# OChicken/GPQHE

Measured on AMD Instinct MI355X. Metric: ciphertext he_mul/sec (RNS core: tensor 30 limbs + key-switch 45 limbs), N=2^16, higher is better.
Workload: dtype u64; 1 GPU; he_mul RNS core, n=2^16, dimA=30, dimB=45, batch=64 ciphertexts per GPU (BASELINE configs[2]); he_rescale has no RNS-domain work in the reference; batch_per_gpu=64, total_batch=64, chunk=32, parallelism=ciphertext-per-GPU x1, no data-path collective, launcher=single process

## Files before the change

### gpqhe_amd/csrc/engine.hip

```cpp
#include "../../include/gpqhe_hip.h"
#include "engine_internal.hpp"
#include "ntt_kernels.hpp"

#include <cmath>
#include <cstdlib>
#include <cstdarg>
#include <cstdio>
#include <cstring>
#include <new>
#include <type_traits>

using namespace gpq;

static thread_local char g_err[512] = "";

int gpq_fail(int code, const char *fmt, ...) {
  va_list ap;
  va_start(ap, fmt);
  vsnprintf(g_err, sizeof g_err, fmt, ap);
  va_end(ap);
  return code;
}
extern "C" const char *gpq_last_error(void) { return g_err; }

// ... 399 lines not shown
    for (int i = 0; i < GPQ_MAX_SLABS; ++i) { if (a.src[i]) a.src[i] += shift; if (a.dst[i]) a.dst[i] += shift; }
    if (evk0) *evk0 += shift;
    if (evk1) *evk1 += shift;
    if (a.zflag) a.zflag += limbs;
  };
  int rc;
  if constexpr (WIDE)
    if (e_wide > lo) { if ((rc = f(TwW{}, a, e_wide - lo))) return rc; advance(e_wide - lo); }
  if (e_split > e_wide) { if ((rc = f(TwS{}, a, e_split - e_wide))) return rc; advance(e_split - e_wide); }
  if (hi > e_split && (rc = f(uint64_t{}, a, hi - e_split))) return rc;
  return GPQ_OK;
}

template <typename F>
static inline void with_nt(unsigned nt, F f) {
  if (nt) f(std::true_type{});
  else f(std::false_type{});
}

template <typename TW_, int LOW_, bool NT_>
struct Mid8Inst { using TW = TW_; static constexpr int LOW = LOW_; static constexpr bool NT = NT_; };
template <typename F>
static int launch_mid8(const gpq_ctx *c, const PassArgs &m, unsigned limbs, const uint64_t **evk0, const uint64_t **evk1, int slot, hipStream_t s, F launch) {
  return for_limb_ranges<true>(c, m, limbs, evk0, evk1, [&](auto tag, const PassArgs &a, unsigned nl) {
    using TW = decltype(tag);
    ProfScope prof(c, slot, s);
    with_nt(a.nt, [&](auto nt) {
      constexpr bool NT = decltype(nt)::value;
      if (c->low9) launch(Mid8Inst<TW, 9, NT>{}, a, nl);
      else launch(Mid8Inst<TW, 8, NT>{}, a, nl);
    });
    return (int)GPQ_OK;
  });
}
template <typename K>
static int launch_mid8(const gpq_ctx *c, const PassArgs &m, unsigned limbs, unsigned polys, int slot, hipStream_t s, K kernel) {
  return launch_mid8(c, m, limbs, nullptr, nullptr, slot, s, [&](auto inst, const PassArgs &a, unsigned nl) {
    hipLaunchKernelGGL(kernel(inst), dim3(c->n >> 11, polys, nl), dim3(CONTIG_WAVES * 64), 0, s, a);
  });
}
template <typename K, typename... Tail>
static int launch_keyswitch_mid8(const gpq_ctx *c, KeyswitchArgs m, unsigned limbs, unsigned polys, int slot, hipStream_t s, K kernel, Tail... tail) {
  return launch_mid8(c, m.p, limbs, &m.evk0, &m.evk1, slot, s, [&](auto inst, const PassArgs &a, unsigned nl) {
    KeyswitchArgs ka{a, m.evk0, m.evk1};
    const dim3 block(CONTIG_WAVES * 64);
    if (polys / 2) hipLaunchKernelGGL(kernel(inst, std::true_type{}), dim3(c->n >> 11, polys / 2, nl), block, 0, s, ka, 0u, tail...);
    if (polys & 1) hipLaunchKernelGGL(kernel(inst, std::false_type{}), dim3(c->n >> 11, 1, nl), block, 0, s, ka, polys - 1, tail...);
  });
}

template <int M1, int EL, bool INV, bool CANON, typename TW, int CW = 8>
int launch_strided_t(const PassArgs &a, unsigned gy, unsigned gz, hipStream_t s) {
  using G = StridedGeom<M1, EL>;
  with_nt(a.nt, [&](auto nt) {
    hipLaunchKernelGGL((strided_pass<M1, EL, INV, CANON, TW, CW, decltype(nt)::value>), dim3((1u << CW) >> G::CB, gy, gz), dim3(G::T), 0, s, a);
  });
  return GPQ_OK;
}

template <bool INV>
int launch_strided(const gpq_ctx *c, const PassArgs &args, unsigned dim, unsigned polys, hipStream_t s) {
  return for_limb_ranges<true>(c, args, dim, nullptr, nullptr, [&](auto tag, const PassArgs &a, unsigned limbs) {
    using TW = decltype(tag);
    ProfScope prof(c, INV ? GPQ_K_STRIDED_INV : GPQ_K_STRIDED_FWD, s);
    switch (c->logn) {
      case 13: return launch_strided_t<5, 4, INV, false, TW>(a, polys * a.nslab, limbs, s);
      case 14: return launch_strided_t<6, 4, INV, false, TW>(a, polys * a.nslab, limbs, s);
      case 15: return launch_strided_t<7, 4, INV, false, TW>(a, polys * a.nslab, limbs, s);
      case 16: return launch_strided_t<8, 4, INV, false, TW>(a, polys * a.nslab, limbs, s);
      case 17:
        return launch_strided_t<8, 4, INV, false, TW, 9>(a, polys * a.nslab, limbs, s);
    }
    return gpq_fail(GPQ_ERR_INVALID, "two-pass NTT needs 13 <= logn <= 17 (got %u)", c->logn);
  });
}

template <bool INV>
int launch_contig(const gpq_ctx *c, const PassArgs &args, unsigned dim, unsigned polys, hipStream_t s) {
  if (args.nslab != 1) return gpq_fail(GPQ_ERR_INVALID, "contig_pass walks one slab");
  return for_limb_ranges<true>(c, args, dim, nullptr, nullptr, [&](auto tag, const PassArgs &a, unsigned limbs) {
    using TW = decltype(tag);
    ProfScope prof(c, INV ? GPQ_K_CONTIG_INV : GPQ_K_CONTIG_FWD, s);
    if (c->low9) {
      const dim3 grid9(c->n >> 11, (polys + CONTIG8_POLYS - 1) / CONTIG8_POLYS, limbs);
      with_nt(a.nt, [&](auto nt) { hipLaunchKernelGGL((contig_pass8<INV, TW, 9, decltype(nt)::value>), grid9, dim3(CONTIG_WAVES * 64), 0, s, a, polys); });
      return (int)GPQ_OK;
    }
    const dim3 grid(c->n >> 12, (polys + CONTIG_POLYS - 1) / CONTIG_POLYS, limbs);
    with_nt(a.nt, [&](auto nt) { hipLaunchKernelGGL((contig_pass<INV, TW, decltype(nt)::value>), grid, dim3(CONTIG_WAVES * 64), 0, s, a, polys); });
    return (int)GPQ_OK;
  });
}

template <bool INV>
int launch_small(const gpq_ctx *c, const PassArgs &args, unsigned dim, unsigned polys, hipStream_t s) {
  return for_limb_ranges<false>(c, args, dim, nullptr, nullptr, [&](auto tag, const PassArgs &a, unsigned limbs) {
    using TW = decltype(tag);
    const dim3 grid(1, polys * a.nslab, limbs);
    ProfScope prof(c, GPQ_K_SMALL, s);
    hipLaunchKernelGGL((small_ntt<INV, TW>), grid, dim3(256), 0, s, a);
    return (int)GPQ_OK;
  });
}

inline bool two_pass(const gpq_ctx *c) { return c->logn > (unsigned)SMALL_MAX_LOGN; }

int after_launch(const char *who) {
  hipError_t e = hipGetLastError();
// ... 574 lines not shown
```

### gpqhe_amd/csrc/ntt_kernels.hpp

```cpp
#pragma once
#include "modarith.hpp"
#include "tables.hpp"

namespace gpq {

template <bool NT> __device__ __forceinline__ uint64_t slab_ld(const uint64_t *p) {
  if constexpr (NT) return __builtin_nontemporal_load(p);
  else return *p;
}
template <bool NT> __device__ __forceinline__ void slab_st(uint64_t *p, uint64_t v) {
  if constexpr (NT) __builtin_nontemporal_store(v, p);
  else *p = v;
}


constexpr int tw_count(int EL, int BHI, int BLO) { return (1 << (EL - BLO)) - (1 << (EL - BHI - 1)); }

constexpr int tw_off(int EL, int BHI, int b) { return (1 << (EL - b - 1)) - (1 << (EL - BHI - 1)); }

template <int EL, int BHI, int B, int BLO, bool UNIFORM, int NTW, typename TW>
__device__ __forceinline__ void load_tw_bits(TW (&tw)[NTW], unsigned ibase, int rs, unsigned logn,
                                             const TW *__restrict__ w) {
  const int sh = rs + B + 1;
  const TW *wp = w + (1u << (logn - sh)) + (UNIFORM ? 0u : (ibase >> sh));
#pragma unroll
  for (int j = 0; j < (1 << (EL - B - 1)); ++j) tw[tw_off(EL, BHI, B) + j] = wp[j];
  if constexpr (B > BLO) load_tw_bits<EL, BHI, B - 1, BLO, UNIFORM>(tw, ibase, rs, logn, w);
}

template <int EL, int BHI, int BLO, bool UNIFORM, typename TW>
__device__ __forceinline__ void load_tw(TW (&tw)[tw_count(EL, BHI, BLO)], unsigned ibase, int rs, unsigned logn,
                                        const TW *__restrict__ w) {
  load_tw_bits<EL, BHI, BHI, BLO, UNIFORM>(tw, ibase, rs, logn, w);
}

template <int S, typename TW>
__device__ __forceinline__ void ct_stage(uint64_t &x, uint64_t &y, const TW &w, const PrimeK &k) { ct_bfly(x, y, w, k); }
template <int S>
__device__ __forceinline__ void ct_stage(uint64_t &x, uint64_t &y, const TwW &w, const PrimeK &k) { ct_bfly_wide<(S & 1) == 0>(x, y, w, k); }

template <int EL, int BHI, int B, int BLO, int RS, int NTW, typename TW>
__device__ __forceinline__ void ct_bits(uint64_t (&x)[1 << EL], const TW (&tw)[NTW], const PrimeK &k) {
#pragma unroll
  for (int e = 0; e < (1 << EL); ++e)
    if (!(e & (1 << B))) ct_stage<RS + B>(x[e], x[e + (1 << B)], tw[tw_off(EL, BHI, B) + (e >> (B + 1))], k);
  if constexpr (B > BLO) ct_bits<EL, BHI, B - 1, BLO, RS>(x, tw, k);
}
template <int EL, int BHI, int BLO, int RS, typename TW>
__device__ __forceinline__ void ct_group(uint64_t (&x)[1 << EL], const TW (&tw)[tw_count(EL, BHI, BLO)],
                                         const PrimeK &k) {
  ct_bits<EL, BHI, BHI, BLO, RS>(x, tw, k);
}

template <bool BOTH_PRODUCT_LEGS, typename TW>
__device__ __forceinline__ void gs_stage(uint64_t &x, uint64_t &y, const TW &w, const PrimeK &k) { gs_bfly(x, y, w, k); }
template <bool BOTH_PRODUCT_LEGS>
__device__ __forceinline__ void gs_stage(uint64_t &x, uint64_t &y, const TwW &w, const PrimeK &k) { gs_bfly_wide<!BOTH_PRODUCT_LEGS>(x, y, w, k); }

template <int EL, int BHI, int B, int NTH, bool CANON_IN, int NTW, typename TW>
__device__ __forceinline__ void gs_bits(uint64_t (&x)[1 << EL], const TW (&tw)[NTW], const PrimeK &k) {
#pragma unroll
  for (int e = 0; e < (1 << EL); ++e)
    if (!(e & (1 << B))) {
      const TW &w = tw[tw_off(EL, BHI, B) + (e >> (B + 1))];
      if ((CANON_IN && NTH < 2) || (NTH > 0 && B > 0 && ((e >> (B > 0 ? B - 1 : 0)) & 1))) gs_stage<true>(x[e], x[e + (1 << B)], w, k);
      else gs_stage<false>(x[e], x[e + (1 << B)], w, k);
    }
// ... 40 lines not shown
template <> struct TwTraits<TwS> {
  __device__ static __forceinline__ const TwS *table(const PassArgs &a, bool inv) { return inv ? a.winvs : a.ws; }
  __device__ static __forceinline__ uint64_t canon_fwd(uint64_t x, const PrimeK &k) { return canon_fold(x, k.p, k.c); }
  __device__ static __forceinline__ uint64_t canon_inv(uint64_t x, const PrimeK &k) { return canon4(x, k); }
  __device__ static __forceinline__ uint64_t inv_from4(uint64_t x, const PrimeK &k) { return csub2(x, k); }
  __device__ static __forceinline__ uint64_t inv_from8(uint64_t x, const PrimeK &k) { return csub2(csub4(x, k), k); }
  __device__ static __forceinline__ uint64_t left(uint64_t x, const PrimeK &k) { return csub2(csub4(x, k), k); }
  __device__ static __forceinline__ uint64_t right(uint64_t x, const PrimeK &) { return x; }
};

template <> struct LastK<TwW> : LastK<TwS> {
  __device__ __forceinline__ explicit LastK(const LimbTab &t) : LastK<TwS>(t) {}
};
__device__ __forceinline__ void gs_last(uint64_t &x, uint64_t &y, const LastK<TwW> &t, const PrimeK &k) {
  const uint64_t s = x + y;
  const uint64_t d = x + k.p4 - y;
  x = csub1(mulmod_split(s, t.ninv, k), k);
  y = csub1(mulmod_split(d, t.winv1_ninv, k), k);
}
template <> struct TwTraits<TwW> {
  __device__ static __forceinline__ const TwW *table(const PassArgs &a, bool inv) { return reinterpret_cast<const TwW *>(inv ? a.winvs : a.ws); }
  __device__ static __forceinline__ uint64_t canon_fwd(uint64_t x, const PrimeK &k) { return canon_fold(x, k.p, k.c); }
  __device__ static __forceinline__ uint64_t canon_inv(uint64_t x, const PrimeK &k) { return canon4(x, k); }
  __device__ static __forceinline__ uint64_t inv_from4(uint64_t x, const PrimeK &) { return x; }
  __device__ static __forceinline__ uint64_t inv_from8(uint64_t x, const PrimeK &k) { return csub4(x, k); }
  __device__ static __forceinline__ uint64_t left(uint64_t x, const PrimeK &k) { return csub4(x, k); }
  __device__ static __forceinline__ uint64_t right(uint64_t x, const PrimeK &) { return x; }
};

__device__ __forceinline__ void zero_watch(uint32_t &m, uint64_t x) {
  const uint32_t t = (uint32_t)x | (uint32_t)(x >> 32);
  m = t < m ? t : m;
}
__device__ __forceinline__ void zero_note(const PassArgs &a, uint32_t m, unsigned poly, unsigned limb_in_launch) {
  if (m == 0 && a.zflag) atomicOr(a.zflag + (size_t)poly * a.zstride + limb_in_launch, 1u);
}

#ifndef GPQ_STRIDED_CB
#define GPQ_STRIDED_CB 4
#endif
template <int M1, int EL>
struct StridedGeom {
  static constexpr int CB = M1 <= 8 ? GPQ_STRIDED_CB : 4;
  static constexpr int C = 1 << CB;
  static constexpr int E = 1 << EL;
  static constexpr int T = 1 << (M1 + CB - EL);
  static constexpr int S2 = M1 - EL;
  static constexpr int BB = S2 > 0 ? S2 - 1 : 0;
  static constexpr int LDS_ELEMS = (1 << (M1 + CB)) + ((S2 > 0) ? (C << S2) : 0);
  __device__ static __forceinline__ unsigned pad(unsigned l) { return l + ((l >> (EL + CB)) << CB); }
};

template <int M1, int EL, bool INV, bool CANON_OUT, typename TW, int CW = 8, bool NT = false>
__global__ __launch_bounds__((StridedGeom<M1, EL>::T)) void strided_pass(PassArgs a) {
  using G = StridedGeom<M1, EL>;
  constexpr int E = G::E;
  constexpr unsigned logn = M1 + CW;
  __shared__ uint64_t lds[G::S2 > 0 ? G::LDS_ELEMS : 1];

  unsigned bx = blockIdx.x, by = blockIdx.y, bz = blockIdx.z;
  if (!INV) {
    const unsigned lin = blockIdx.x + gridDim.x * (blockIdx.y + gridDim.y * blockIdx.z), tot = gridDim.x * gridDim.y * gridDim.z;
    const unsigned logical = (lin & 7) * (tot >> 3) + (lin >> 3);
    bx = logical % gridDim.x; by = (logical / gridDim.x) % gridDim.y; bz = logical / (gridDim.x * gridDim.y);
  }
  const unsigned limb = a.limb0 + bz;
  const LimbTab &tab = a.tabs[limb];
  const PrimeK k = pin_consts(tab.k);
  const LastK<TW> last(tab);
  const TW *__restrict__ wt = TwTraits<TW>::table(a, INV) + ((size_t)limb << logn);
  const unsigned slab = by % a.nslab, poly = by / a.nslab;
  const size_t off = (size_t)poly * a.poly_stride + ((size_t)bz << logn);
  const uint64_t *__restrict__ src = a.src[slab] + off;
  uint64_t *__restrict__ dst = a.dst[slab] + off;

  const unsigned tid = threadIdx.x;
  constexpr int CB = G::CB;
  const unsigned col = (bx << CB) + (tid & (G::C - 1));
  const unsigned q = tid >> CB;
  const unsigned iA = (q << CW) + col, iB = (q << (EL + CW)) + col;
  constexpr unsigned strideA = 1u << (G::S2 + CW), strideB = 1u << CW;
  uint64_t x[E];
  TW twB[tw_count(EL, G::BB, 0)];

  if (!INV) {
    TW twA[tw_count(EL, EL - 1, 0)];
#pragma unroll
    for (int e = 0; e < E; ++e) x[e] = slab_ld<NT>(&src[iA + e * strideA]);
    load_tw<EL, EL - 1, 0, true>(twA, iA, G::S2 + CW, logn, wt);
    if (G::S2 > 0) load_tw<EL, G::BB, 0, false>(twB, iB, CW, logn, wt);
    ct_group<EL, EL - 1, 0, G::S2 + CW>(x, twA, k);
    if (G::S2 > 0) {
#pragma unroll
      for (int e = 0; e < E; ++e) lds[G::pad(tid + e * G::T)] = x[e];
      __syncthreads();
#pragma unroll
      for (int e = 0; e < E; ++e) x[e] = lds[G::pad((q << (EL + CB)) + (e << CB) + (tid & (G::C - 1)))];
      ct_group<EL, G::BB, 0, CW>(x, twB, k);
#pragma unroll
      for (int e = 0; e < E; ++e) slab_st<NT>(&dst[iB + e * strideB], CANON_OUT ? TwTraits<TW>::canon_fwd(x[e], k) : x[e]);
    } else {
#pragma unroll
      for (int e = 0; e < E; ++e) slab_st<NT>(&dst[iA + e * strideA], CANON_OUT ? TwTraits<TW>::canon_fwd(x[e], k) : x[e]);
    }
  } else {
    TW twA[tw_count(EL, (EL > 1 ? EL - 2 : 0), 0)];
    if (G::S2 > 0) {
#pragma unroll
      for (int e = 0; e < E; ++e) x[e] = slab_ld<NT>(&src[iB + e * strideB]);
      load_tw<EL, G::BB, 0, false>(twB, iB, CW, logn, wt);
      if (EL > 1) load_tw<EL, (EL > 1 ? EL - 2 : 0), 0, true>(twA, iA, G::S2 + CW, logn, wt);
      gs_group<EL, G::BB, 0>(x, twB, k);
#pragma unroll
      for (int e = 0; e < E; ++e) lds[G::pad((q << (EL + CB)) + (e << CB) + (tid & (G::C - 1)))] = x[e];
      __syncthreads();
#pragma unroll
      for (int e = 0; e < E; ++e) x[e] = lds[G::pad(tid + e * G::T)];
    } else {
#pragma unroll
      for (int e = 0; e < E; ++e) x[e] = slab_ld<NT>(&src[iA + e * strideA]);
      if (EL > 1) load_tw<EL, (EL > 1 ? EL - 2 : 0), 0, true>(twA, iA, G::S2 + CW, logn, wt);
    }
    if (EL > 1) gs_group<EL, (EL > 1 ? EL - 2 : 0), 0>(x, twA, k);
#pragma unroll
    for (int e = 0; e < E / 2; ++e) gs_last(x[e], x[e + E / 2], last, k);
#pragma unroll
    for (int e = 0; e < E; ++e) slab_st<NT>(&dst[iA + e * strideA], x[e]);
  }
}

constexpr int CONTIG_WAVES = 4;
constexpr int CONTIG_LDS_PER_WAVE = 1024 + 64;

__device__ __forceinline__ void wave_lds_sync() {
  __builtin_amdgcn_fence(__ATOMIC_RELEASE, "wavefront");
  __builtin_amdgcn_wave_barrier();
  __builtin_amdgcn_fence(__ATOMIC_ACQUIRE, "wavefront");
}

struct ContigLane {
  unsigned j, blk, hbase, lbase;
  uint64_t *lds;
  __device__ __forceinline__ ContigLane(uint64_t *wave_lds) {
    const unsigned lane = threadIdx.x & 63;
    j = lane & 15; blk = lane >> 4;
    hbase = (blk << 8) + j;
    lbase = (blk << 8) + (j << 4);
    lds = wave_lds;
  }
  __device__ static __forceinline__ unsigned pad(unsigned l) { return l + (l >> 4); }
  __device__ __forceinline__ void h_to_l(uint64_t (&x)[16]) const {
#pragma unroll
    for (int e = 0; e < 16; ++e) lds[pad(hbase + 16 * e)] = x[e];
    wave_lds_sync();
#pragma unroll
    for (int e = 0; e < 16; ++e) x[e] = lds[pad(lbase + e)];
    wave_lds_sync();
  }
  __device__ __forceinline__ void l_to_h(uint64_t (&x)[16]) const {
#pragma unroll
    for (int e = 0; e < 16; ++e) lds[pad(lbase + e)] = x[e];
    wave_lds_sync();
#pragma unroll
    for (int e = 0; e < 16; ++e) x[e] = lds[pad(hbase + 16 * e)];
    wave_lds_sync();
  }
};

template <typename TW>
struct ContigTw {
  TW t[15];
  __device__ __forceinline__ void load_h(const ContigLane &ln, unsigned wave0, unsigned logn, const TW *__restrict__ w) {
    load_tw<4, 3, 0, false>(t, wave0 + ln.hbase, 4, logn, w);
  }
  __device__ __forceinline__ void load_l(const ContigLane &ln, unsigned wave0, unsigned logn, const TW *__restrict__ w) {
    load_tw<4, 3, 0, false>(t, wave0 + ln.lbase, 0, logn, w);
  }
};

template <bool NT> __device__ __forceinline__ void load_h(uint64_t (&x)[16], const uint64_t *__restrict__ p, const ContigLane &ln) {
// ... 162 lines not shown
    for (int e = 0; e < 8; ++e) x[e] = lds[pad2(mk + (e << MB))];
    wave_lds_sync();
  }
  __device__ __forceinline__ void m_to_h(uint64_t (&x)[8]) const {
#pragma unroll
    for (int e = 0; e < 8; ++e) lds[pad1(mk + (e << MB))] = x[e];
    wave_lds_sync();
#pragma unroll
    for (int e = 0; e < 8; ++e) x[e] = lds[pad1(hk + (e << JB))];
    wave_lds_sync();
  }
  __device__ __forceinline__ void l_to_h(uint64_t (&x)[8]) const {
#pragma unroll
    for (int e = 0; e < 8; ++e) lds[pad2(lk + e)] = x[e];
    wave_lds_sync();
#pragma unroll
    for (int e = 0; e < 8; ++e) x[e] = lds[pad2(hk + (e << JB))];
    wave_lds_sync();
  }
  __device__ __forceinline__ void h_to_l(uint64_t (&x)[8]) const {
#pragma unroll
    for (int e = 0; e < 8; ++e) lds[pad2(hk + (e << JB))] = x[e];
    wave_lds_sync();
#pragma unroll
    for (int e = 0; e < 8; ++e) x[e] = lds[pad2(lk + e)];
    wave_lds_sync();
  }
  __device__ __forceinline__ void load_l(uint64_t (&x)[8], const uint64_t *__restrict__ p) const {
    const ulonglong2 *v = reinterpret_cast<const ulonglong2 *>(p + lk);
#pragma unroll
    for (int e = 0; e < 4; ++e) { ulonglong2 t = v[e]; x[2 * e] = t.x; x[2 * e + 1] = t.y; }
  }
  template <typename TW> __device__ static __forceinline__ void ct_h(uint64_t (&x)[8], const TW (&t)[7], const PrimeK &k) { ct_group<3, 2, 0, LOW - 3>(x, t, k); }
  template <typename TW> __device__ static __forceinline__ void ct_m(uint64_t (&x)[8], const TW (&t)[7], const PrimeK &k) { ct_group<3, 2, 0, LOW - 6>(x, t, k); }
  template <typename TW> __device__ static __forceinline__ void ct_l(uint64_t (&x)[8], const TW (&u)[tw_count(3, LHI, 0)], const PrimeK &k) { ct_group<3, LHI, 0, 0>(x, u, k); }
  template <typename TW> __device__ static __forceinline__ void gs_hm(uint64_t (&x)[8], const TW (&t)[7], const PrimeK &k) { gs_group<3, 2, 0>(x, t, k); }
  template <typename TW> __device__ static __forceinline__ void gs_l(uint64_t (&x)[8], const TW (&u)[tw_count(3, LHI, 0)], const PrimeK &k) { gs_group<3, LHI, 0>(x, u, k); }
  template <typename TW> __device__ static __forceinline__ void gs_l_canon(uint64_t (&x)[8], const TW (&u)[tw_count(3, LHI, 0)], const PrimeK &k) { gs_group<3, LHI, 0, true>(x, u, k); }
};

template <int LOW, bool NT>
struct Lane8N : Lane8<LOW> {
  using Lane8<LOW>::hk;
  using Lane8<LOW>::JB;
  __device__ __forceinline__ Lane8N(uint64_t *wave_lds) : Lane8<LOW>(wave_lds) {}
  __device__ __forceinline__ void load_h(uint64_t (&x)[8], const uint64_t *__restrict__ p) const {
#pragma unroll
    for (int e = 0; e < 8; ++e) x[e] = slab_ld<NT>(&p[hk + (e << JB)]);
  }
  __device__ __forceinline__ void store_h(uint64_t *__restrict__ p, const uint64_t (&x)[8]) const {
#pragma unroll
    for (int e = 0; e < 8; ++e) slab_st<NT>(&p[hk + (e << JB)], x[e]);
  }
};

template <typename TW, int LOW>
struct Tw8 {
  using L8 = Lane8<LOW>;
  TW t[7];
  TW u[tw_count(3, L8::LHI, 0)];
  __device__ __forceinline__ void load_h(const L8 &ln, unsigned wave0, unsigned logn, const TW *__restrict__ w) {
    load_tw<3, 2, 0, false>(t, wave0 + ln.hk, LOW - 3, logn, w);
  }
  __device__ __forceinline__ void load_m(const L8 &ln, unsigned wave0, unsigned logn, const TW *__restrict__ w) {
    load_tw<3, 2, 0, false>(t, wave0 + ln.mk, LOW - 6, logn, w);
  }
  __device__ __forceinline__ void load_l(const L8 &ln, unsigned wave0, unsigned logn, const TW *__restrict__ w) {
    load_tw<3, L8::LHI, 0, false>(u, wave0 + ln.lk, 0, logn, w);
  }
};

#ifndef GPQ_MID8_MINWAVES
#define GPQ_MID8_MINWAVES 3
#endif
template <typename TW, int LOW, bool NT>
struct Mid8 {
  using TT = TwTraits<TW>;
  using L8 = Lane8N<LOW, NT>;
  L8 ln;
  const unsigned wave0, logn, limb;
  const size_t toff;
  const PrimeK k;
  const TW *__restrict__ wf, *__restrict__ wi;
  Tw8<TW, LOW> tw;
  __device__ __forceinline__ Mid8(uint64_t *lds, const PassArgs &a)
      : ln(lds + (threadIdx.x >> 6) * LANE8_LDS_PER_WAVE), wave0((blockIdx.x * CONTIG_WAVES + (threadIdx.x >> 6)) << 9), logn(a.logn), limb(a.limb0 + blockIdx.z),
        toff((size_t)limb << a.logn), k(pin_consts(a.tabs[limb].k)), wf(TT::table(a, false) + toff), wi(TT::table(a, true) + toff) {}
  __device__ __forceinline__ size_t off(const PassArgs &a, unsigned poly) const { return (size_t)poly * a.poly_stride + ((size_t)blockIdx.z << a.logn) + wave0; }
  __device__ __forceinline__ void load_first(uint64_t (&x)[8], const uint64_t *__restrict__ p) { ln.load_h(x, p); tw.load_h(ln, wave0, logn, wf); }
  __device__ __forceinline__ void load(uint64_t (&x)[8], const uint64_t *__restrict__ p) const { ln.load_h(x, p); }
  template <typename... X> __device__ __forceinline__ void forward(X &...x) {
    (L8::ct_h(x, tw.t, k), ...);
    tw.load_m(ln, wave0, logn, wf);
    ((ln.h_to_m(x), L8::ct_m(x, tw.t, k)), ...);
    tw.load_l(ln, wave0, logn, wf);
    ((ln.m_to_l(x), L8::ct_l(x, tw.u, k)), ...);
  }
  __device__ __forceinline__ void load_inverse_l() { tw.load_l(ln, wave0, logn, wi); }
  template <typename... X> __device__ __forceinline__ void inverse(X &...x) {
    ((L8::gs_l(x, tw.u, k), ln.l_to_m(x)), ...);
    tw.load_m(ln, wave0, logn, wi);
    ((L8::gs_hm(x, tw.t, k), ln.m_to_h(x)), ...);
    tw.load_h(ln, wave0, logn, wi);
  }
  __device__ __forceinline__ void finish(uint64_t (&x)[8]) const { L8::gs_hm(x, tw.t, k); }
};

template <typename TW, int LOW, bool NT = false>
__global__ __launch_bounds__(CONTIG_WAVES * 64, GPQ_MID8_MINWAVES) void tensor_mid8(PassArgs a) {
  using TT = TwTraits<TW>;
  __shared__ uint64_t lds[CONTIG_WAVES * LANE8_LDS_PER_WAVE];
  uint64_t a0[8], a1[8], b0[8], b1[8];
  Mid8<TW, LOW, NT> s(lds, a);
  const size_t off = s.off(a, blockIdx.y);
  const PrimeK &k = s.k;
  s.load_first(a0, a.src[0] + off);
  s.load(b0, a.src[2] + off);
  s.load(a1, a.src[1] + off);
  s.load(b1, a.src[3] + off);
  s.forward(a0, b0, a1, b1);
  s.load_inverse_l();
  uint64_t d1[8];
#pragma unroll
  for (int e = 0; e < 8; ++e) {
    const uint64_t u0 = TT::left(a0[e], k), u1 = TT::left(a1[e], k);
    const uint64_t v0 = TT::right(b0[e], k), v1 = TT::right(b1[e], k);
    a0[e] = TT::inv_from4(mulmod_lazy(u0, v0, k), k);
    d1[e] = TT::inv_from8(mulmod_lazy(u0, v1, k) + mulmod_lazy(u1, v0, k), k);
    a1[e] = TT::inv_from4(mulmod_lazy(u1, v1, k), k);
  }
  s.inverse(a0, d1, a1);
  s.finish(a0); s.ln.store_h(a.dst[0] + off, a0);
  s.finish(d1); s.ln.store_h(a.dst[1] + off, d1);
  s.finish(a1); s.ln.store_h(a.dst[2] + off, a1);
}

template <typename TW, int LOW, bool NT = false>
__global__ __launch_bounds__(CONTIG_WAVES * 64, GPQ_MID8_MINWAVES) void tensor_sq_mid8(PassArgs a) {
  using TT = TwTraits<TW>;
  __shared__ uint64_t lds[CONTIG_WAVES * LANE8_LDS_PER_WAVE];
  uint64_t a0[8], a1[8];
  Mid8<TW, LOW, NT> s(lds, a);
  const size_t off = s.off(a, blockIdx.y);
  const PrimeK &k = s.k;
  s.load_first(a0, a.src[0] + off);
  s.load(a1, a.src[1] + off);
  s.forward(a0, a1);
  s.load_inverse_l();
  uint64_t d1[8];
#pragma unroll
  for (int e = 0; e < 8; ++e) {
    const uint64_t u0 = TT::left(a0[e], k), u1 = TT::left(a1[e], k);
    const uint64_t v0 = TT::right(a0[e], k), v1 = TT::right(a1[e], k);
    const uint64_t cross = mulmod_lazy(u0, v1, k);
    a0[e] = TT::inv_from4(mulmod_lazy(u0, v0, k), k);
    d1[e] = TT::inv_from8(cross + cross, k);
    a1[e] = TT::inv_from4(mulmod_lazy(u1, v1, k), k);
  }
  s.inverse(a0, d1, a1);
  s.finish(a0); s.ln.store_h(a.dst[0] + off, a0);
  s.finish(d1); s.ln.store_h(a.dst[1] + off, d1);
  s.finish(a1); s.ln.store_h(a.dst[2] + off, a1);
}

template <typename TW, int LOW, bool NT = false>
__global__ __launch_bounds__(CONTIG_WAVES * 64, 4) void polymul_mid8(PassArgs a) {
  using TT = TwTraits<TW>;
  __shared__ uint64_t lds[CONTIG_WAVES * LANE8_LDS_PER_WAVE];
  uint64_t x[8], y[8];
  Mid8<TW, LOW, NT> s(lds, a);
  const size_t off = s.off(a, blockIdx.y);
  const PrimeK &k = s.k;
  s.load_first(x, a.src[0] + off);
  s.load(y, a.src[1] + off);
  s.forward(x, y);
  s.load_inverse_l();
#pragma unroll
  for (int e = 0; e < 8; ++e) x[e] = TT::inv_from4(mulmod_lazy(TT::left(x[e], k), TT::right(y[e], k), k), k);
  s.inverse(x);
  s.finish(x); s.ln.store_h(a.dst[0] + off, x);
}

template <typename TW, int LOW, bool NT = false>
__global__ __launch_bounds__(CONTIG_WAVES * 64, 3) void mulpt_mid8(PassArgs a) {
  using TT = TwTraits<TW>;
  __shared__ uint64_t lds[CONTIG_WAVES * LANE8_LDS_PER_WAVE];
  uint64_t m[8], x[8], y[8];
  Mid8<TW, LOW, NT> s(lds, a);
  const size_t off = s.off(a, blockIdx.y);
  const PrimeK &k = s.k;
  s.load_first(m, a.src[0] + off);
  s.load(x, a.src[1] + off);
  s.load(y, a.src[2] + off);
  s.forward(m, x, y);
  s.load_inverse_l();
#pragma unroll
  for (int e = 0; e < 8; ++e) {
    const uint64_t u = TT::left(m[e], k);
    x[e] = TT::inv_from4(mulmod_lazy(u, TT::right(x[e], k), k), k);
    y[e] = TT::inv_from4(mulmod_lazy(u, TT::right(y[e], k), k), k);
  }
  s.inverse(x, y);
  s.finish(x); s.ln.store_h(a.dst[0] + off, x);
  s.finish(y); s.ln.store_h(a.dst[1] + off, y);
}

#define GPQ_KEYSWITCH_PRODUCTS()                                  \
  s.ln.load_l(e0, ka.evk0 + koff);                                \
  s.ln.load_l(e1, ka.evk1 + koff);                                \
  s.load_inverse_l();                                             \
  uint64_t y0[8], y1[8];                                          \
  _Pragma("unroll") for (int e = 0; e < 8; ++e) {                 \
    const uint64_t u0 = TT::right(x0[e], k);                      \
    x0[e] = TT::inv_from4(mulmod_lazy(u0, e0[e], k), k);          \
    y0[e] = TT::inv_from4(mulmod_lazy(u0, e1[e], k), k);          \
  }                                                               \
  if constexpr (TWO) {                                            \
    _Pragma("unroll") for (int e = 0; e < 8; ++e) {               \
      const uint64_t u1 = TT::right(x1[e], k);                    \
      x1[e] = TT::inv_from4(mulmod_lazy(u1, e0[e], k), k);        \
      y1[e] = TT::inv_from4(mulmod_lazy(u1, e1[e], k), k);        \
    }                                                             \
  }
template <bool TWO, typename S>
__device__ __forceinline__ void keyswitch_back(S &s, const PassArgs &a, uint64_t (&x0)[8], uint64_t (&y0)[8], uint64_t (&x1)[8], uint64_t (&y1)[8], size_t off0, size_t off1) {
  if constexpr (TWO) s.inverse(x0, y0, x1, y1);
  else s.inverse(x0, y0);
  s.finish(x0); s.ln.store_h(a.dst[0] + off0, x0);
  s.finish(y0); s.ln.store_h(a.dst[1] + off0, y0);
  if constexpr (TWO) {
    s.finish(x1); s.ln.store_h(a.dst[0] + off1, x1);
    s.finish(y1); s.ln.store_h(a.dst[1] + off1, y1);
  }
}

template <typename TW, int LOW, bool TWO = true, bool NT = false>
__global__ __launch_bounds__(CONTIG_WAVES * 64, TWO ? 4 : 3) void keyswitch_mid8x2(KeyswitchArgs ka, unsigned first) {
  using TT = TwTraits<TW>;
  __shared__ uint64_t lds[CONTIG_WAVES * LANE8_LDS_PER_WAVE];
  const PassArgs &a = ka.p;
  Mid8<TW, LOW, NT> s(lds, a);
  const unsigned wave0 = s.wave0;
  const PrimeK &k = s.k;
  const unsigned p0 = first + 2 * blockIdx.y;
  const size_t off0 = s.off(a, p0);
  const size_t off1 = TWO ? off0 + a.poly_stride : off0;
  const size_t koff = ((size_t)blockIdx.z << a.logn) + wave0;
  uint64_t x0[8], x1[8], e0[8], e1[8];
  s.load_first(x0, a.src[0] + off0);
  if constexpr (TWO) { s.load(x1, a.src[0] + off1); s.forward(x0, x1); }
  else s.forward(x0);
  GPQ_KEYSWITCH_PRODUCTS();
  keyswitch_back<TWO>(s, a, x0, y0, x1, y1, off0, off1);
}

__device__ __forceinline__ unsigned automorphism_src(unsigned j, unsigned logn, unsigned g) {
  const unsigned mask2n = (2u << logn) - 1;
  const unsigned e = (((__brev(j) >> (32 - logn)) << 1) | 1u) * g & mask2n;
  return __brev(e >> 1) >> (32 - logn);
}

template <typename TW, int LOW, bool TWO = true, bool NT = false>
__global__ __launch_bounds__(CONTIG_WAVES * 64, TWO ? 4 : 3) void keyswitch_rot_mid8x2(KeyswitchArgs ka, unsigned first, unsigned g) {
  using TT = TwTraits<TW>;
  using L8 = Lane8N<LOW, NT>;
  __shared__ uint64_t lds[CONTIG_WAVES * LANE8_LDS_PER_WAVE];
  const PassArgs &a = ka.p;
  Mid8<TW, LOW, NT> s(lds, a);
  const unsigned wave0 = s.wave0;
  const PrimeK &k = s.k;
  const unsigned p0 = first + 2 * blockIdx.y;
  const size_t off0 = (size_t)p0 * a.poly_stride + ((size_t)blockIdx.z << a.logn) + wave0;
  const size_t off1 = TWO ? off0 + a.poly_stride : off0;
  const size_t koff = ((size_t)blockIdx.z << a.logn) + wave0;
  const L8 &ln = s.ln;
  const unsigned src0 = automorphism_src(wave0, a.logn, g) & ~511u;
  const size_t soff0 = off0 - wave0 + src0, soff1 = off1 - wave0 + src0;
  unsigned sl[8];
#pragma unroll
  for (int e = 0; e < 8; ++e) sl[e] = automorphism_src(wave0 + ln.lk + e, a.logn, g) & 511u;
  auto gather = [&](uint64_t (&x)[8], size_t soff) {
    ln.load_h(x, a.src[0] + soff);
#pragma unroll
    for (int e = 0; e < 8; ++e) ln.lds[L8::pad2(ln.hk + (e << L8::JB))] = x[e];
    wave_lds_sync();
#pragma unroll
    for (int e = 0; e < 8; ++e) x[e] = ln.lds[L8::pad2(sl[e])];
    wave_lds_sync();
  };
  uint64_t x0[8], x1[8], e0[8], e1[8];
  gather(x0, soff0);
  if constexpr (TWO) gather(x1, soff1);
  GPQ_KEYSWITCH_PRODUCTS();
  keyswitch_back<TWO>(s, a, x0, y0, x1, y1, off0, off1);
}
#undef GPQ_KEYSWITCH_PRODUCTS

__global__ __launch_bounds__(256) void automorphism_gather(const uint64_t *__restrict__ src, uint64_t *__restrict__ dst, unsigned logn, unsigned g) {
  const unsigned j = blockIdx.x * 256 + threadIdx.x;
  if (j >= (1u << logn)) return;
  const size_t row = (size_t)blockIdx.y << logn;
  dst[row + j] = src[row + automorphism_src(j, logn, g)];
}

typedef unsigned long long v2u64 __attribute__((ext_vector_type(2)));
struct GemvMacArgs {
  const LimbTab *tabs;
  const uint64_t *r0, *r1;
  const uint64_t *diag;
  uint64_t *acc0, *acc1;
  const uint2 *terms;
  unsigned nterms, polys, dim, logn;
};
template <bool NT>
__device__ __forceinline__ v2u64 gemv_ld16(const v2u64 *p) {
  if constexpr (NT) return __builtin_nontemporal_load(p);
  else return *p;
}
template <int BT, bool NT>
__global__ __launch_bounds__(256) void gemv_mac(GemvMacArgs a) {
  const PrimeK k = pin_consts(a.tabs[blockIdx.z].k);
// ... 278 lines not shown
```

### gpqhe_amd/csrc/tables.hpp

```cpp
#pragma once
#include "modarith.hpp"

namespace gpq {

struct LimbTab {
  PrimeK k;
  uint64_t ninv;
  uint64_t winv1_ninv;
  TwS ninv_s, winv1_ninv_s;
};

constexpr unsigned GEMV_NOT_LIVE = 0xffffffffu;

#define GPQ_MAX_SLABS 4
struct PassArgs {
  const LimbTab *tabs;
  const uint64_t *w;
  const uint64_t *winv;
  const TwS *ws;
  const TwS *winvs;
  const uint64_t *src[GPQ_MAX_SLABS];
  uint64_t *dst[GPQ_MAX_SLABS];
  unsigned long long poly_stride;
  unsigned logn;
  unsigned limb0;
  unsigned nslab;
  unsigned *zflag;
  unsigned zstride;
  unsigned nt;
};

}
```

Before: 7831 he_mul/s.

## Use buffer-resource addressing and precomputed magic division in NTT slab kernels

Replaces flat 64-bit pointer loads/stores in the strided and mid8 NTT kernels with AMD buffer resource descriptors, using 32-bit lane/element offsets to cut 64-bit address arithmetic and VGPR pressure. It also replaces runtime div/mod in block-index decoding with host-precomputed multiply-shift division constants. Risks include compiler codegen differences, a bound check on grid size, and the rotation kernel staying on the old path.

```diff
diff --git a/gpqhe_amd/csrc/engine.hip b/gpqhe_amd/csrc/engine.hip
--- a/gpqhe_amd/csrc/engine.hip
+++ b/gpqhe_amd/csrc/engine.hip
@@ -475,8 +475,10 @@
 template <int M1, int EL, bool INV, bool CANON, typename TW, int CW = 8>
 int launch_strided_t(const PassArgs &a, unsigned gy, unsigned gz, hipStream_t s) {
   using G = StridedGeom<M1, EL>;
+  if ((unsigned long long)gy * gz > (1ull << 31)) return gpq_fail(GPQ_ERR_INVALID, "strided pass: %u x %u workgroup rows are beyond the kernel's index math", gy, gz);
+  const StridedGrid g{div_by(gy, (unsigned long long)gy * gz), div_by(a.nslab, gy)};
   with_nt(a.nt, [&](auto nt) {
-    hipLaunchKernelGGL((strided_pass<M1, EL, INV, CANON, TW, CW, decltype(nt)::value>), dim3((1u << CW) >> G::CB, gy, gz), dim3(G::T), 0, s, a);
+    hipLaunchKernelGGL((strided_pass<M1, EL, INV, CANON, TW, CW, decltype(nt)::value>), dim3((1u << CW) >> G::CB, gy, gz), dim3(G::T), 0, s, a, g);
   });
   return GPQ_OK;
 }
diff --git a/gpqhe_amd/csrc/ntt_kernels.hpp b/gpqhe_amd/csrc/ntt_kernels.hpp
--- a/gpqhe_amd/csrc/ntt_kernels.hpp
+++ b/gpqhe_amd/csrc/ntt_kernels.hpp
@@ -13,6 +13,33 @@
   else *p = v;
 }
 
+#ifndef GPQ_BUFFER_ADDR
+#define GPQ_BUFFER_ADDR 1
+#endif
+typedef unsigned v2u32 __attribute__((ext_vector_type(2)));
+struct SlabRow {
+  __amdgpu_buffer_rsrc_t r;
+  __device__ __forceinline__ SlabRow(const uint64_t *slab, size_t row_off, unsigned logn)
+      : r(__builtin_amdgcn_make_buffer_rsrc(const_cast<uint64_t *>(slab + row_off), 0, 8u << logn, 0x00020000)) {}
+};
+template <bool BUF> __device__ __forceinline__ auto slab_row(const uint64_t *slab, size_t row_off, unsigned logn) {
+  if constexpr (BUF) return SlabRow(slab, row_off, logn);
+  else return slab + row_off;
+}
+template <bool BUF> __device__ __forceinline__ auto slab_row(uint64_t *slab, size_t row_off, unsigned logn) {
+  if constexpr (BUF) return SlabRow(slab, row_off, logn);
+  else return slab + row_off;
+}
+template <bool NT> __device__ __forceinline__ uint64_t slab_ld(SlabRow row, unsigned lane, unsigned elem) {
+  const v2u32 v = __builtin_amdgcn_raw_buffer_load_b64(row.r, lane * 8, elem * 8, NT ? 2 : 0);
+  return (uint64_t)v.x | ((uint64_t)v.y << 32);
+}
+template <bool NT> __device__ __forceinline__ void slab_st(SlabRow row, unsigned lane, unsigned elem, uint64_t w) {
+  __builtin_amdgcn_raw_buffer_store_b64(v2u32{(unsigned)w, (unsigned)(w >> 32)}, row.r, lane * 8, elem * 8, NT ? 2 : 0);
+}
+template <bool NT> __device__ __forceinline__ uint64_t slab_ld(const uint64_t *row, unsigned lane, unsigned elem) { return slab_ld<NT>(&row[lane + elem]); }
+template <bool NT> __device__ __forceinline__ void slab_st(uint64_t *row, unsigned lane, unsigned elem, uint64_t w) { slab_st<NT>(&row[lane + elem], w); }
+__device__ __forceinline__ unsigned div_u(unsigned t, const DivU &d) { return (__umulhi(t, d.mul) >> d.shift) + (t & d.pass); }
 
 constexpr int tw_count(int EL, int BHI, int BLO) { return (1 << (EL - BLO)) - (1 << (EL - BHI - 1)); }
 
@@ -159,7 +186,7 @@
 };
 
 template <int M1, int EL, bool INV, bool CANON_OUT, typename TW, int CW = 8, bool NT = false>
-__global__ __launch_bounds__((StridedGeom<M1, EL>::T)) void strided_pass(PassArgs a) {
+__global__ __launch_bounds__((StridedGeom<M1, EL>::T)) void strided_pass(PassArgs a, StridedGrid g) {
   using G = StridedGeom<M1, EL>;
   constexpr int E = G::E;
   constexpr unsigned logn = M1 + CW;
@@ -169,17 +196,28 @@
   if (!INV) {
     const unsigned lin = blockIdx.x + gridDim.x * (blockIdx.y + gridDim.y * blockIdx.z), tot = gridDim.x * gridDim.y * gridDim.z;
     const unsigned logical = (lin & 7) * (tot >> 3) + (lin >> 3);
+#if GPQ_BUFFER_ADDR
+    const unsigned t = logical >> (CW - G::CB);
+    bx = logical & ((1u << (CW - G::CB)) - 1); bz = div_u(t, g.gy); by = t - bz * gridDim.y;
+#else
     bx = logical % gridDim.x; by = (logical / gridDim.x) % gridDim.y; bz = logical / (gridDim.x * gridDim.y);
+#endif
   }
   const unsigned limb = a.limb0 + bz;
   const LimbTab &tab = a.tabs[limb];
   const PrimeK k = pin_consts(tab.k);
   const LastK<TW> last(tab);
   const TW *__restrict__ wt = TwTraits<TW>::table(a, INV) + ((size_t)limb << logn);
+#if GPQ_BUFFER_ADDR
+  const unsigned poly = div_u(by, g.nslab), slab = by - poly * a.nslab;
+  const size_t off = (size_t)poly * a.poly_stride + ((size_t)bz << logn);
+  const SlabRow dst(a.dst[slab], off, logn), src = INV ? dst : SlabRow(a.src[slab], off, logn);
+#else
   const unsigned slab = by % a.nslab, poly = by / a.nslab;
   const size_t off = (size_t)poly * a.poly_stride + ((size_t)bz << logn);
   const uint64_t *__restrict__ src = a.src[slab] + off;
   uint64_t *__restrict__ dst = a.dst[slab] + off;
+#endif
 
   const unsigned tid = threadIdx.x;
   constexpr int CB = G::CB;
@@ -193,7 +231,7 @@
   if (!INV) {
     TW twA[tw_count(EL, EL - 1, 0)];
 #pragma unroll
-    for (int e = 0; e < E; ++e) x[e] = slab_ld<NT>(&src[iA + e * strideA]);
+    for (int e = 0; e < E; ++e) x[e] = slab_ld<NT>(src, iA, e * strideA);
     load_tw<EL, EL - 1, 0, true>(twA, iA, G::S2 + CW, logn, wt);
     if (G::S2 > 0) load_tw<EL, G::BB, 0, false>(twB, iB, CW, logn, wt);
     ct_group<EL, EL - 1, 0, G::S2 + CW>(x, twA, k);
@@ -205,16 +243,16 @@
       for (int e = 0; e < E; ++e) x[e] = lds[G::pad((q << (EL + CB)) + (e << CB) + (tid & (G::C - 1)))];
       ct_group<EL, G::BB, 0, CW>(x, twB, k);
 #pragma unroll
-      for (int e = 0; e < E; ++e) slab_st<NT>(&dst[iB + e * strideB], CANON_OUT ? TwTraits<TW>::canon_fwd(x[e], k) : x[e]);
+      for (int e = 0; e < E; ++e) slab_st<NT>(dst, iB, e * strideB, CANON_OUT ? TwTraits<TW>::canon_fwd(x[e], k) : x[e]);
     } else {
 #pragma unroll
-      for (int e = 0; e < E; ++e) slab_st<NT>(&dst[iA + e * strideA], CANON_OUT ? TwTraits<TW>::canon_fwd(x[e], k) : x[e]);
+      for (int e = 0; e < E; ++e) slab_st<NT>(dst, iA, e * strideA, CANON_OUT ? TwTraits<TW>::canon_fwd(x[e], k) : x[e]);
     }
   } else {
     TW twA[tw_count(EL, (EL > 1 ? EL - 2 : 0), 0)];
     if (G::S2 > 0) {
 #pragma unroll
-      for (int e = 0; e < E; ++e) x[e] = slab_ld<NT>(&src[iB + e * strideB]);
+      for (int e = 0; e < E; ++e) x[e] = slab_ld<NT>(src, iB, e * strideB);
       load_tw<EL, G::BB, 0, false>(twB, iB, CW, logn, wt);
       if (EL > 1) load_tw<EL, (EL > 1 ? EL - 2 : 0), 0, true>(twA, iA, G::S2 + CW, logn, wt);
       gs_group<EL, G::BB, 0>(x, twB, k);
@@ -225,14 +263,14 @@
       for (int e = 0; e < E; ++e) x[e] = lds[G::pad(tid + e * G::T)];
     } else {
 #pragma unroll
-      for (int e = 0; e < E; ++e) x[e] = slab_ld<NT>(&src[iA + e * strideA]);
+      for (int e = 0; e < E; ++e) x[e] = slab_ld<NT>(src, iA, e * strideA);
       if (EL > 1) load_tw<EL, (EL > 1 ? EL - 2 : 0), 0, true>(twA, iA, G::S2 + CW, logn, wt);
     }
     if (EL > 1) gs_group<EL, (EL > 1 ? EL - 2 : 0), 0>(x, twA, k);
 #pragma unroll
     for (int e = 0; e < E / 2; ++e) gs_last(x[e], x[e + E / 2], last, k);
 #pragma unroll
-    for (int e = 0; e < E; ++e) slab_st<NT>(&dst[iA + e * strideA], x[e]);
+    for (int e = 0; e < E; ++e) slab_st<NT>(dst, iA, e * strideA, x[e]);
   }
 }
 
@@ -501,6 +539,16 @@
 #pragma unroll
     for (int e = 0; e < 8; ++e) slab_st<NT>(&p[hk + (e << JB)], x[e]);
   }
+  __device__ __forceinline__ void load_h(uint64_t (&x)[8], const SlabRow &p, unsigned w0) const {
+#pragma unroll
+    for (int e = 0; e < 8; ++e) x[e] = slab_ld<NT>(p, w0 + hk, e << JB);
+  }
+  __device__ __forceinline__ void store_h(const SlabRow &p, const uint64_t (&x)[8], unsigned w0) const {
+#pragma unroll
+    for (int e = 0; e < 8; ++e) slab_st<NT>(p, w0 + hk, e << JB, x[e]);
+  }
+  __device__ __forceinline__ void load_h(uint64_t (&x)[8], const uint64_t *__restrict__ p, unsigned) const { load_h(x, p); }
+  __device__ __forceinline__ void store_h(uint64_t *__restrict__ p, const uint64_t (&x)[8], unsigned) const { store_h(p, x); }
 };
 
 template <typename TW, int LOW>
@@ -522,7 +570,7 @@
 #ifndef GPQ_MID8_MINWAVES
 #define GPQ_MID8_MINWAVES 3
 #endif
-template <typename TW, int LOW, bool NT>
+template <typename TW, int LOW, bool NT, bool BUF = (GPQ_BUFFER_ADDR != 0)>
 struct Mid8 {
   using TT = TwTraits<TW>;
   using L8 = Lane8N<LOW, NT>;
@@ -535,9 +583,14 @@
   __device__ __forceinline__ Mid8(uint64_t *lds, const PassArgs &a)
       : ln(lds + (threadIdx.x >> 6) * LANE8_LDS_PER_WAVE), wave0((blockIdx.x * CONTIG_WAVES + (threadIdx.x >> 6)) << 9), logn(a.logn), limb(a.limb0 + blockIdx.z),
         toff((size_t)limb << a.logn), k(pin_consts(a.tabs[limb].k)), wf(TT::table(a, false) + toff), wi(TT::table(a, true) + toff) {}
-  __device__ __forceinline__ size_t off(const PassArgs &a, unsigned poly) const { return (size_t)poly * a.poly_stride + ((size_t)blockIdx.z << a.logn) + wave0; }
-  __device__ __forceinline__ void load_first(uint64_t (&x)[8], const uint64_t *__restrict__ p) { ln.load_h(x, p); tw.load_h(ln, wave0, logn, wf); }
-  __device__ __forceinline__ void load(uint64_t (&x)[8], const uint64_t *__restrict__ p) const { ln.load_h(x, p); }
+  __device__ __forceinline__ size_t off(const PassArgs &a, unsigned poly) const {
+    if constexpr (BUF) return (size_t)poly * a.poly_stride + ((size_t)blockIdx.z << a.logn);
+    else return (size_t)poly * a.poly_stride + ((size_t)blockIdx.z << a.logn) + wave0;
+  }
+  __device__ __forceinline__ auto row(const uint64_t *slab, size_t o) const { return slab_row<BUF>(slab, o, logn); }
+  __device__ __forceinline__ auto row(uint64_t *slab, size_t o) const { return slab_row<BUF>(slab, o, logn); }
+  template <typename R> __device__ __forceinline__ void load_first(uint64_t (&x)[8], const R &p) { ln.load_h(x, p, wave0); tw.load_h(ln, wave0, logn, wf); }
+  template <typename R> __device__ __forceinline__ void load(uint64_t (&x)[8], const R &p) const { ln.load_h(x, p, wave0); }
   template <typename... X> __device__ __forceinline__ void forward(X &...x) {
     (L8::ct_h(x, tw.t, k), ...);
     tw.load_m(ln, wave0, logn, wf);
@@ -563,10 +616,10 @@
   Mid8<TW, LOW, NT> s(lds, a);
   const size_t off = s.off(a, blockIdx.y);
   const PrimeK &k = s.k;
-  s.load_first(a0, a.src[0] + off);
-  s.load(b0, a.src[2] + off);
-  s.load(a1, a.src[1] + off);
-  s.load(b1, a.src[3] + off);
+  s.load_first(a0, s.row(a.src[0], off));
+  s.load(b0, s.row(a.src[2], off));
+  s.load(a1, s.row(a.src[1], off));
+  s.load(b1, s.row(a.src[3], off));
   s.forward(a0, b0, a1, b1);
   s.load_inverse_l();
   uint64_t d1[8];
@@ -579,9 +632,9 @@
     a1[e] = TT::inv_from4(mulmod_lazy(u1, v1, k), k);
   }
   s.inverse(a0, d1, a1);
-  s.finish(a0); s.ln.store_h(a.dst[0] + off, a0);
-  s.finish(d1); s.ln.store_h(a.dst[1] + off, d1);
-  s.finish(a1); s.ln.store_h(a.dst[2] + off, a1);
+  s.finish(a0); s.ln.store_h(s.row(a.dst[0], off), a0, s.wave0);
+  s.finish(d1); s.ln.store_h(s.row(a.dst[1], off), d1, s.wave0);
+  s.finish(a1); s.ln.store_h(s.row(a.dst[2], off), a1, s.wave0);
 }
 
 template <typename TW, int LOW, bool NT = false>
@@ -592,8 +645,8 @@
   Mid8<TW, LOW, NT> s(lds, a);
   const size_t off = s.off(a, blockIdx.y);
   const PrimeK &k = s.k;
-  s.load_first(a0, a.src[0] + off);
-  s.load(a1, a.src[1] + off);
+  s.load_first(a0, s.row(a.src[0], off));
+  s.load(a1, s.row(a.src[1], off));
   s.forward(a0, a1);
   s.load_inverse_l();
   uint64_t d1[8];
@@ -607,9 +660,9 @@
     a1[e] = TT::inv_from4(mulmod_lazy(u1, v1, k), k);
   }
   s.inverse(a0, d1, a1);
-  s.finish(a0); s.ln.store_h(a.dst[0] + off, a0);
-  s.finish(d1); s.ln.store_h(a.dst[1] + off, d1);
-  s.finish(a1); s.ln.store_h(a.dst[2] + off, a1);
+  s.finish(a0); s.ln.store_h(s.row(a.dst[0], off), a0, s.wave0);
+  s.finish(d1); s.ln.store_h(s.row(a.dst[1], off), d1, s.wave0);
+  s.finish(a1); s.ln.store_h(s.row(a.dst[2], off), a1, s.wave0);
 }
 
 template <typename TW, int LOW, bool NT = false>
@@ -620,14 +673,14 @@
   Mid8<TW, LOW, NT> s(lds, a);
   const size_t off = s.off(a, blockIdx.y);
   const PrimeK &k = s.k;
-  s.load_first(x, a.src[0] + off);
-  s.load(y, a.src[1] + off);
+  s.load_first(x, s.row(a.src[0], off));
+  s.load(y, s.row(a.src[1], off));
   s.forward(x, y);
   s.load_inverse_l();
 #pragma unroll
   for (int e = 0; e < 8; ++e) x[e] = TT::inv_from4(mulmod_lazy(TT::left(x[e], k), TT::right(y[e], k), k), k);
   s.inverse(x);
-  s.finish(x); s.ln.store_h(a.dst[0] + off, x);
+  s.finish(x); s.ln.store_h(s.row(a.dst[0], off), x, s.wave0);
 }
 
 template <typename TW, int LOW, bool NT = false>
@@ -635,12 +688,12 @@
   using TT = TwTraits<TW>;
   __shared__ uint64_t lds[CONTIG_WAVES * LANE8_LDS_PER_WAVE];
   uint64_t m[8], x[8], y[8];
-  Mid8<TW, LOW, NT> s(lds, a);
+  Mid8<TW, LOW, NT, GPQ_BUFFER_ADDR && sizeof(TW) == 8> s(lds, a);
   const size_t off = s.off(a, blockIdx.y);
   const PrimeK &k = s.k;
-  s.load_first(m, a.src[0] + off);
-  s.load(x, a.src[1] + off);
-  s.load(y, a.src[2] + off);
+  s.load_first(m, s.row(a.src[0], off));
+  s.load(x, s.row(a.src[1], off));
+  s.load(y, s.row(a.src[2], off));
   s.forward(m, x, y);
   s.load_inverse_l();
 #pragma unroll
@@ -650,8 +703,8 @@
     y[e] = TT::inv_from4(mulmod_lazy(u, TT::right(y[e], k), k), k);
   }
   s.inverse(x, y);
-  s.finish(x); s.ln.store_h(a.dst[0] + off, x);
-  s.finish(y); s.ln.store_h(a.dst[1] + off, y);
+  s.finish(x); s.ln.store_h(s.row(a.dst[0], off), x, s.wave0);
+  s.finish(y); s.ln.store_h(s.row(a.dst[1], off), y, s.wave0);
 }
 
 #define GPQ_KEYSWITCH_PRODUCTS()                                  \
@@ -675,11 +728,11 @@
 __device__ __forceinline__ void keyswitch_back(S &s, const PassArgs &a, uint64_t (&x0)[8], uint64_t (&y0)[8], uint64_t (&x1)[8], uint64_t (&y1)[8], size_t off0, size_t off1) {
   if constexpr (TWO) s.inverse(x0, y0, x1, y1);
   else s.inverse(x0, y0);
-  s.finish(x0); s.ln.store_h(a.dst[0] + off0, x0);
-  s.finish(y0); s.ln.store_h(a.dst[1] + off0, y0);
+  s.finish(x0); s.ln.store_h(s.row(a.dst[0], off0), x0, s.wave0);
+  s.finish(y0); s.ln.store_h(s.row(a.dst[1], off0), y0, s.wave0);
   if constexpr (TWO) {
-    s.finish(x1); s.ln.store_h(a.dst[0] + off1, x1);
-    s.finish(y1); s.ln.store_h(a.dst[1] + off1, y1);
+    s.finish(x1); s.ln.store_h(s.row(a.dst[0], off1), x1, s.wave0);
+    s.finish(y1); s.ln.store_h(s.row(a.dst[1], off1), y1, s.wave0);
   }
 }
 
@@ -696,8 +749,8 @@
   const size_t off1 = TWO ? off0 + a.poly_stride : off0;
   const size_t koff = ((size_t)blockIdx.z << a.logn) + wave0;
   uint64_t x0[8], x1[8], e0[8], e1[8];
-  s.load_first(x0, a.src[0] + off0);
-  if constexpr (TWO) { s.load(x1, a.src[0] + off1); s.forward(x0, x1); }
+  s.load_first(x0, s.row(a.src[0], off0));
+  if constexpr (TWO) { s.load(x1, s.row(a.src[0], off1)); s.forward(x0, x1); }
   else s.forward(x0);
   GPQ_KEYSWITCH_PRODUCTS();
   keyswitch_back<TWO>(s, a, x0, y0, x1, y1, off0, off1);
@@ -715,7 +768,7 @@
   using L8 = Lane8N<LOW, NT>;
   __shared__ uint64_t lds[CONTIG_WAVES * LANE8_LDS_PER_WAVE];
   const PassArgs &a = ka.p;
-  Mid8<TW, LOW, NT> s(lds, a);
+  Mid8<TW, LOW, NT, false> s(lds, a);
   const unsigned wave0 = s.wave0;
   const PrimeK &k = s.k;
   const unsigned p0 = first + 2 * blockIdx.y;
diff --git a/gpqhe_amd/csrc/tables.hpp b/gpqhe_amd/csrc/tables.hpp
--- a/gpqhe_amd/csrc/tables.hpp
+++ b/gpqhe_amd/csrc/tables.hpp
@@ -30,4 +30,18 @@
   unsigned nt;
 };
 
+struct DivU { unsigned mul, shift, pass; };
+inline DivU div_by(unsigned d, unsigned long long bound) {
+  if (d <= 1) return DivU{0, 0, ~0u};
+  unsigned b = 1, l = 1;
+  while (b < 31 && (1ull << b) < bound) ++b;
+  while ((1u << l) < d) ++l;
+  const unsigned k = b + l < 32 ? 32 : b + l;
+  return DivU{(unsigned)((((unsigned long long)1 << k) + d - 1) / d), k - 32, 0};
 }
+struct StridedGrid {
+  DivU gy;
+  DivU nslab;
+};
+
+}
```

Measured after the change: 7904 he_mul/s (median of 6 runs). Within noise of the previous version (+0.9%).
